# yjcaimeow/pointnerf

Hardware: AMD Instinct MI355X
Metric: Mray-samples/sec at 800x800, K=8, 2M neural points; PSNR delta vs ref (higher is better)
Workload: dtype fp32h2

## Files before the change

pointnerf_amd/csrc/aggregate_x3.hip:

```cpp
#include "agg_common.h"


namespace pnr {
namespace {

constexpr int kXT = 64;
constexpr int kXTS = kXT / kKN;
constexpr int kHidPlane = 32 * 64 * 16;
constexpr int kHidTile = 2 * kHidPlane;
constexpr int kXG = 34;
constexpr int kPG = 8;
constexpr int kPlaneX = kXG * kXT * 16;
constexpr int kPlaneP = kPG * kXT * 16;
constexpr int kP1Pitch = kHid + 4;

template <bool H>
struct XL {
  static constexpr int NPL = H ? 2 : 3;
  static constexpr int NPW = H ? 2 : 3;
  static constexpr unsigned kOne = H ? 0x3C00u : 0x3F80u;
  static constexpr int OffPE = NPL * kPlaneX;
  static constexpr int OffEx = OffPE + NPL * kPlaneP;
  static constexpr int NWB = H ? 3 : 2;
  static constexpr int OffWt = OffEx + 2 * 8 * kXT * 4;
  static constexpr int OffPr = OffWt + NWB * kXT * 4;
  static constexpr int OffSf = OffPr + 2 * kXT * 4;
  static constexpr int OffAp = OffSf + NWB * kXTS * 4;
  static constexpr int OffWa = OffAp + 4 * kXT * 4;
  static constexpr int OffH4 = OffWa + kHid * 4;
  static constexpr int OffTq = OffH4 + (H ? kXT * kP1Pitch * 4 : 0);
  static constexpr size_t Lds = (size_t)OffTq + 16;
  static_assert(OffSf % 16 == 0 && OffWa % 16 == 0 && OffH4 % 16 == 0, "16-B aligned LDS arrays");
  static_assert(kXT * kP1Pitch * 4 <= NPL * kPlaneX, "parked P1 fits the layer-input area");
  static_assert(Lds <= 160 * 1024, "LDS budget");
};

constexpr int kProducerPrio = 3;
constexpr int kStoreWindowPrio = 0;

typedef float f32x2n __attribute__((ext_vector_type(2)));
typedef float f32x4n __attribute__((ext_vector_type(4)));

struct X3Args {
  pnr_points pts;
  pnr_samples s;
  pnr_mlp w;
  SplitW wx;
  const float* p1;
  float* hid;
  int32_t* vmask;
  float* out_feat;
  float* out_weight;
  float* out_conf;
  int32_t* tile_ctr;
  pnr_agg_saved sv;
};

__device__ __forceinline__ bool xcd_mode(int64_t nt) { return nt >= 2 * (int64_t)gridDim.x + 16; }
__device__ __forceinline__ int64_t xcd_lo(int64_t nt, int x) { return nt * x / 8; }
__device__ __forceinline__ int64_t xcd_nb(int x) { return ((int)gridDim.x - x + 7) / 8; }

__device__ __forceinline__ int64_t first_tile(int64_t nt) {
  if (!xcd_mode(nt)) return blockIdx.x;
  return xcd_lo(nt, blockIdx.x & 7) + (blockIdx.x >> 3);
}

__device__ __forceinline__ int64_t take_tile(const X3Args& A, int64_t nt) {
  if (!xcd_mode(nt)) return (int64_t)gridDim.x + atomicAdd(A.tile_ctr, 1);
  const int x0 = blockIdx.x & 7;
  for (int i = 0; i < 8; ++i) {
    const int x = (x0 + i) & 7;
    const int64_t t = xcd_lo(nt, x) + xcd_nb(x) + atomicAdd(A.tile_ctr + x, 1);
    if (t < xcd_lo(nt, x + 1)) return t;
  }
  return nt;
}

__device__ __forceinline__ __amdgpu_buffer_rsrc_t rsrc(const void* base) {
  return __builtin_amdgcn_make_buffer_rsrc(const_cast<void*>(base), 0, 0x7fffffff, 0x00020000);
}

template <bool H, int NTK = 8>
__device__ __forceinline__ void load_w(uint4 (&a)[2][XL<H>::NPW], __amdgpu_buffer_rsrc_t rs, int voff, int t) {
  constexpr int NPW = XL<H>::NPW;
#pragma unroll
  for (int T = 0; T < 2; ++T)
#pragma unroll
    for (int pl = 0; pl < NPW; ++pl)
      a[T][pl] = __builtin_bit_cast(
          uint4, __builtin_amdgcn_raw_buffer_load_b128(
                     rs, voff + pl * 1024, (t * NTK + T) * NPW * 1024, 0));
}

template <bool H>
struct WRing {
  static constexpr int kWD = 3;
  uint4 a[kWD][2][XL<H>::NPW];
};

template <bool H, int NTK = 8>
__device__ __forceinline__ void prime(WRing<H>& w, __amdgpu_buffer_rsrc_t rs, int voff) {
#pragma unroll
  for (int d = 0; d < WRing<H>::kWD; ++d) load_w<H, NTK>(w.a[d], rs, voff, d);
}

template <bool H, int NTK = 8, bool ACC2 = false, bool ZACC = false>
__device__ __forceinline__ void layer(f32x16 (&acc)[4], f32x16 (&corr)[4], WRing<H>& w, __amdgpu_buffer_rsrc_t rs,
                                      int voff, const char* planes, int pstride, int nsteps, int lane) {
  static_assert(ACC2 || !ZACC, "zero-start accumulators: with two accumulator sets only");
  static_assert(H || !ACC2, "two accumulator sets: the f16 split only");
  constexpr int NPL = XL<H>::NPL, NPW = XL<H>::NPW, kWD = WRing<H>::kWD;
  const int c = lane & 31, h = lane >> 5;
  const char* base = planes + (h * kXT + c) * 16;
  auto ldb = [&](int t, int pt, uint4 (&bb)[NPL]) {
#pragma unroll
    for (int pl = 0; pl < NPL; ++pl)
      bb[pl] = *reinterpret_cast<const uint4*>(base + pl * pstride + (2 * t * kXT + 32 * pt) * 16);
  };
  constexpr int BD = H ? 2 : 1;
  uint4 b[BD][2][NPL];
#pragma unroll
  for (int sl = 0; sl < BD; ++sl) {
    const int t0 = sl < nsteps ? sl : nsteps - 1;
    ldb(t0, 0, b[sl][0]);
    ldb(t0, 1, b[sl][1]);
  }
  auto mm = [&](int pt, const uint4& av0, const uint4& av1, const uint4& bv, bool to_corr = false, bool zc = false) {
    if constexpr (ACC2) {
      f32x16 (&d)[4] = to_corr ? corr : acc;
      const f32x16 z = {0.f};
      d[2 * pt] = mfma_f16(av0, bv, zc ? z : d[2 * pt]);
      d[2 * pt + 1] = mfma_f16(av1, bv, zc ? z : d[2 * pt + 1]);
    } else if constexpr (H) {
      acc[2 * pt] = mfma_f16(av0, bv, acc[2 * pt]);
      acc[2 * pt + 1] = mfma_f16(av1, bv, acc[2 * pt + 1]);
    } else {
      acc[2 * pt] = mfma_bf16(av0, bv, acc[2 * pt]);
      acc[2 * pt + 1] = mfma_bf16(av1, bv, acc[2 * pt + 1]);
    }
  };
  auto wl = [&](uint4 (&a)[2][NPW], int pl, int tw) {
#pragma unroll
    for (int T = 0; T < 2; ++T)
      a[T][pl] = __builtin_bit_cast(
          uint4, __builtin_amdgcn_raw_buffer_load_b128(
                     rs, voff + pl * 1024, (tw * NTK + T) * NPW * 1024, 0));
  };
  auto bl = [&](int bs, int tn, int pt, int pl) {
    b[bs][pt][pl] = *reinterpret_cast<const uint4*>(base + pl * pstride + (2 * tn * kXT + 32 * pt) * 16);
  };
  uint4 scl[2];
  auto scale_next = [&](const uint4 (&an)[2][NPW], int T) {
    if constexpr (!ACC2) scl[T] = f16x8_scale2048(an[T][0]);
  };
  if constexpr (H) {
    scale_next(w.a[0], 0);
    scale_next(w.a[0], 1);
  }
  auto step_h = [&](uint4 (&a)[2][NPW], const uint4 (&an)[2][NPW], int t, int bs, bool first = false) {
    const int tn = t + BD < nsteps ? t + BD : nsteps - 1;
    const uint4 s0 = ACC2 ? a[0][0] : scl[0], s1 = ACC2 ? a[1][0] : scl[1];
#pragma unroll
    for (int pt = 0; pt < 2; ++pt) {
      mm(pt, s0, s1, b[bs][pt][0], false, first && ZACC);
      __builtin_amdgcn_sched_barrier(0);
      mm(pt, a[0][1], a[1][1], b[bs][pt][0], true, first);
      __builtin_amdgcn_sched_barrier(0);
      if (pt == 1) wl(a, 1, t + kWD);
      if (pt == 0) scale_next(an, 0);
      bl(bs, tn, pt, 0);
      __builtin_amdgcn_sched_barrier(0);
      mm(pt, a[0][0], a[1][0], b[bs][pt][1], true);
      __builtin_amdgcn_sched_barrier(0);
      bl(bs, tn, pt, 1);
      if (pt == 0) scale_next(an, 1);
      if (pt == 1) wl(a, 0, t + kWD);
      __builtin_amdgcn_sched_barrier(0);
    }
  };
  auto step = [&](uint4 (&a)[2][NPW], const uint4 (&an)[2][NPW], int t, int bs) {
    if constexpr (H) {
      step_h(a, an, t, bs);
    } else {
      const int tn = t + BD < nsteps ? t + BD : nsteps - 1;
#pragma unroll
      for (int pt = 0; pt < 2; ++pt) {
        mm(pt, a[0][2], a[1][2], b[bs][pt][0]);
        __builtin_amdgcn_sched_barrier(0);
        if (pt == 1) wl(a, 2, t + kWD);
        __builtin_amdgcn_sched_barrier(0);
        mm(pt, a[0][1], a[1][1], b[bs][pt][1]);
        mm(pt, a[0][0], a[1][0], b[bs][pt][2]);
        __builtin_amdgcn_sched_barrier(0);
        bl(bs, tn, pt, 2);
        __builtin_amdgcn_sched_barrier(0);
        mm(pt, a[0][1], a[1][1], b[bs][pt][0]);
        __builtin_amdgcn_sched_barrier(0);
        if (pt == 1) wl(a, 1, t + kWD);
        __builtin_amdgcn_sched_barrier(0);
        mm(pt, a[0][0], a[1][0], b[bs][pt][1]);
        __builtin_amdgcn_sched_barrier(0);
        bl(bs, tn, pt, 1);
        __builtin_amdgcn_sched_barrier(0);
        mm(pt, a[0][0], a[1][0], b[bs][pt][0]);
        __builtin_amdgcn_sched_barrier(0);
        bl(bs, tn, pt, 0);
        if (pt == 1) wl(a, 0, t + kWD);
        __builtin_amdgcn_sched_barrier(0);
      }
    }
  };
  constexpr int U = (BD == 2 && kWD % 2) ? 2 * kWD : kWD;
  constexpr int P = ACC2 ? 1 : 0;
  if constexpr (ACC2) step_h(w.a[0], w.a[1 % kWD], 0, 0, true);
  int t = P;
#pragma unroll 1
  for (; t + U <= nsteps; t += U) {
#pragma unroll
    for (int d = 0; d < U; ++d) step(w.a[(d + P) % kWD], w.a[(d + P + 1) % kWD], t + d, (d + P) % BD);
  }
#pragma unroll
  for (int d = 0; d < U - 1; ++d)
    if (t + d < nsteps) step(w.a[(d + P) % kWD], w.a[(d + P + 1) % kWD], t + d, (d + P) % BD);
}

template <bool H, int NTK = 8>
__device__ __forceinline__ void layer(f32x16 (&acc)[4], WRing<H>& w, __amdgpu_buffer_rsrc_t rs, int voff,
                                      const char* planes, int pstride, int nsteps, int lane) {
  layer<H, NTK, false>(acc, acc, w, rs, voff, planes, pstride, nsteps, lane);
}

__device__ __forceinline__ float fold2(float main, float corr) { return fmaf(main, 2048.f, corr); }

__device__ __forceinline__ void lrelu_splith(float x0, float x1, float k, float ks, unsigned& hi, unsigned& lo) {
  typedef float f2 __attribute__((ext_vector_type(2)));
  const f2 x = {x0, x1};
  const f2 Y = __builtin_elementwise_max(x * k, x * ks);
  asm volatile(
      "v_fma_mixlo_f16 %0, %2, %4, 0\n\t"
      "v_fma_mixhi_f16 %0, %3, %4, 0\n\t"
      "v_fma_mixlo_f16 %1, %0, %5, %2 op_sel_hi:[1,0,0]\n\t"
      "v_fma_mixhi_f16 %1, %0, %5, %3 op_sel:[1,0,0] op_sel_hi:[1,0,0]"
      : "=&v"(hi), "=&v"(lo)
      : "v"(Y.x), "v"(Y.y), "s"(0x1p-11f), "s"(-2048.f));
}

template <bool H, bool ACC2 = false>
__device__ __forceinline__ void store_act(const f32x16 (&acc)[4], const f32x16 (&corr)[4], char* planes, float s,
                                          float mul, int lane, int T0, int pstride = kPlaneX) {
  const int c = lane & 31, h = lane >> 5;
  if constexpr (H) {
    const float k = 2048.f * mul, ks = k * s;
#pragma unroll
    for (int pt = 0; pt < 2; ++pt)
#pragma unroll
      for (int T = 0; T < 2; ++T)
#pragma unroll
        for (int q = 0; q < 4; ++q) {
          float v[4];
#pragma unroll
          for (int i = 0; i < 4; ++i)
            v[i] = ACC2 ? fold2(acc[2 * pt + T][4 * q + i], corr[2 * pt + T][4 * q + i]) : acc[2 * pt + T][4 * q + i];
          unsigned a0, a1, b0, b1;
          lrelu_splith(v[0], v[1], k, ks, a0, a1);
          lrelu_splith(v[2], v[3], k, ks, b0, b1);
          char* d = planes + ((4 * (T0 + T) + q) * kXT + 32 * pt + c) * 16 + 8 * h;
          *reinterpret_cast<uint2*>(d) = make_uint2(a0, b0);
          *reinterpret_cast<uint2*>(d + pstride) = make_uint2(a1, b1);
        }
    return;
  }
#pragma unroll
  for (int pt = 0; pt < 2; ++pt)
#pragma unroll
    for (int T = 0; T < 2; ++T)
#pragma unroll
      for (int q = 0; q < 4; ++q) {
        const f32x16& v = acc[2 * pt + T];
        unsigned a0, a1, a2, b0, b1, b2;
        split2(fmaxf(v[4 * q], s * v[4 * q]), fmaxf(v[4 * q + 1], s * v[4 * q + 1]), a0, a1, a2);
        split2(fmaxf(v[4 * q + 2], s * v[4 * q + 2]), fmaxf(v[4 * q + 3], s * v[4 * q + 3]), b0, b1, b2);
        char* d = planes + ((4 * (T0 + T) + q) * kXT + 32 * pt + c) * 16 + 8 * h;
        *reinterpret_cast<uint2*>(d) = make_uint2(a0, b0);
        *reinterpret_cast<uint2*>(d + kPlaneX) = make_uint2(a1, b1);
        *reinterpret_cast<uint2*>(d + 2 * kPlaneX) = make_uint2(a2, b2);
      }
}

template <bool H>
__device__ __forceinline__ void store_act(const f32x16 (&acc)[4], char* planes, float s, float mul, int lane,
                                          int T0, int pstride = kPlaneX) {
  store_act<H, false>(acc, acc, planes, s, mul, lane, T0, pstride);
}

template <bool H>
__device__ __forceinline__ void acc_init(f32x16 (&acc)[4], const float* bias, float inv_scale, int lane, int T0) {
  if constexpr (H) {
    const int h = lane >> 5;
#pragma unroll
    for (int T = 0; T < 2; ++T)
#pragma unroll
      for (int q = 0; q < 4; ++q) {
        const float4 b = *reinterpret_cast<const float4*>(bias + 32 * (T0 + T) + 8 * q + 4 * h);
        const float v[4] = {b.x * inv_scale, b.y * inv_scale, b.z * inv_scale, b.w * inv_scale};
#pragma unroll
        for (int i = 0; i < 4; ++i) {
          acc[T][4 * q + i] = v[i];
          acc[2 + T][4 * q + i] = v[i];
        }
      }
  } else {
#pragma unroll
    for (int i = 0; i < 4; ++i) acc[i] = (f32x16){0.f};
  }
}
constexpr int kBiasSteps(bool H) { return H ? 16 : 17; }

template <bool H>
__device__ __forceinline__ void store_group(char* planes, int pstride, int g, int pair, const float (&v)[8]) {
  if constexpr (H) {
    uint4 p0, p1;
    splith(v[0], v[1], p0.x, p1.x);
    splith(v[2], v[3], p0.y, p1.y);
    splith(v[4], v[5], p0.z, p1.z);
    splith(v[6], v[7], p0.w, p1.w);
    char* d = planes + (g * kXT + pair) * 16;
    *reinterpret_cast<uint4*>(d) = p0;
    *reinterpret_cast<uint4*>(d + pstride) = p1;
    return;
  }
  uint4 p0, p1, p2;
  split2(v[0], v[1], p0.x, p1.x, p2.x);
  split2(v[2], v[3], p0.y, p1.y, p2.y);
  split2(v[4], v[5], p0.z, p1.z, p2.z);
  split2(v[6], v[7], p0.w, p1.w, p2.w);
  char* d = planes + (g * kXT + pair) * 16;
  *reinterpret_cast<uint4*>(d) = p0;
  *reinterpret_cast<uint4*>(d + pstride) = p1;
  *reinterpret_cast<uint4*>(d + 2 * pstride) = p2;
}

struct GatherState {
  int64_t tile;
  int64_t row;
  int pid;
  float sw[3], sp[3];
  int64_t dmap;
  bool active;
};

__device__ __forceinline__ void gather_row(const X3Args& A, int64_t tile, int lane, GatherState& g) {
  const int64_t v = tile * kXTS + (lane >> 3);
  g.tile = tile;
  g.active = v < eff_n(A.s);
  g.row = g.active ? sample_row(A.s, v) : 0;
}

__device__ __forceinline__ void gather_sample(const X3Args& A, int lane, GatherState& g) {
  const int k = lane & 7, K = A.s.K;
  g.pid = (g.active && k < K) ? A.s.pidx[g.row * K + k] : -1;
#pragma unroll
  for (int a = 0; a < 3; ++a) {
    g.sw[a] = g.active ? A.s.sample_w[g.row * 3 + a] : 0.f;
    g.sp[a] = g.active ? A.s.sample_p[g.row * 3 + a] : 0.f;
  }
  g.dmap = A.s.dir_map ? (int64_t)A.s.dir_map[g.row] : g.row;
}

template <bool H, bool TR = false>
__device__ __forceinline__ void gather(const X3Args& A, const GatherState& g, int nb, int nw, char* lds, int pw, int lane,
                                       float (&dr6)[6]) {
  using L = XL<H>;
  float Rw[9];
#pragma unroll
  for (int i = 0; i < 9; ++i) Rw[i] = A.w.rw2c ? A.w.rw2c[i] : (i % 4 == 0 ? 1.f : 0.f);
  float cam_c[3] = {0.f, 0.f, 0.f}, cam_R[9] = {1.f, 0.f, 0.f, 0.f, 1.f, 0.f, 0.f, 0.f, 1.f};
  if (!A.pts.pers) {
#pragma unroll
    for (int i = 0; i < 3; ++i) cam_c[i] = A.pts.campos[i];
#pragma unroll
    for (int i = 0; i < 9; ++i) cam_R[i] = A.pts.camrot[i];
  }
  const int j = lane >> 3, k = lane & 7;
  const int K = A.s.K;
  const bool active = g.active;
  const int64_t row = g.row;
  const bool valid = g.pid >= 0;
  const int64_t prow = valid ? g.pid : (active && k < K ? 0 : -1);
  float sw[3], sp[3], vd[3] = {0.f, 0.f, 0.f};
#pragma unroll
  for (int a = 0; a < 3; ++a) {
    sw[a] = g.sw[a];
    sp[a] = g.sp[a];
  }
  const int64_t drow = active ? g.dmap / A.s.dir_div : 0;
  if (active && pw == 0) {
#pragma unroll
    for (int a = 0; a < 3; ++a) vd[a] = A.s.dirs[drow * 3 + a];
  }
  float pw3[3] = {0.f, 0.f, 0.f}, pp[3] = {0.f, 0.f, 0.f}, col[3] = {0.f, 0.f, 0.f}, pdir[3] = {0.f, 0.f, 0.f};
  float cf = 1.f;
  if (valid) {
#pragma unroll
    for (int a = 0; a < 3; ++a) pw3[a] = A.pts.xyz[prow * 3 + a];
    if (pw == 0) {
#pragma unroll
      for (int a = 0; a < 3; ++a) {
        col[a] = A.pts.color ? A.pts.color[prow * 3 + a] : 0.f;
        pdir[a] = A.pts.dir ? A.pts.dir[prow * 3 + a] : 0.f;
      }
    }
    if (A.pts.pers) {
#pragma unroll
      for (int a = 0; a < 3; ++a) pp[a] = A.pts.pers[prow * 3 + a];
    } else {
      pair_pers(A.pts, A.s, drow, pw3, cam_c, cam_R, pp);
    }
  }
  if (pw == 0 && A.pts.conf && prow >= 0) cf = A.pts.conf[prow];
  float d6[6];
  d6[0] = pw3[0] - sw[0];
  d6[1] = pw3[1] - sw[1];
  d6[2] = pw3[2] - sw[2];
  d6[3] = pp[0] * pp[2] - sp[0] * sp[2];
  d6[4] = pp[1] * pp[2] - sp[1] * sp[2];
  d6[5] = pp[2] - sp[2];
  mat3(Rw, d6, dr6);
  dr6[3] = d6[3];
  dr6[4] = d6[4];
  dr6[5] = d6[5];
  if (A.pts.rw2c) rot_point(A.pts.rw2c, prow, d6, dr6);
  if (pw == 0) {
    const float nrm = sqrtf(d6[0] * d6[0] + d6[1] * d6[1] + d6[2] * d6[2]);
    const float wl = valid ? 1.f / fmaxf(nrm, 1e-6f) : 0.f;
    const float wsum = xor8_sum(wl);
    const float wn = wl / fmaxf(wsum, 1e-8f);
    const float confc = fminf(fmaxf(cf, 1e-4f), 1.f);
    const bool samp_valid = xor8_sum(valid ? 1.f : 0.f) > 0.f;
    float vrot[3], drot[3];
    mat3(Rw, vd, vrot);
    mat3(Rw, pdir, drot);
    if (A.pts.rw2c) {
      rot_point(A.pts.rw2c, prow, pdir, drot);
      rot_point(A.pts.rw2c, active ? slot0_point(A.s, row) : 0, vd, vrot);
    }
    const float dot = drot[0] * vrot[0] + drot[1] * vrot[1] + drot[2] * vrot[2];
    const float ex[8] = {col[0], col[1], col[2], drot[0] - vrot[0], drot[1] - vrot[1], drot[2] - vrot[2], dot, 1.f};
    float* exL = reinterpret_cast<float*>(lds + L::OffEx) + nb * 8 * kXT;
#pragma unroll
    for (int e = 0; e < 8; ++e) exL[e * kXT + lane] = ex[e];
    reinterpret_cast<float*>(lds + L::OffWt)[nw * kXT + lane] = wn * confc;
    reinterpret_cast<int*>(lds + L::OffPr)[nb * kXT + lane] = valid ? (int)prow : -1;
    if (k == 0) reinterpret_cast<int*>(lds + L::OffSf)[nw * kXTS + j] = active && samp_valid;
    if (active && k < K) {
      if (A.out_weight) A.out_weight[row * K + k] = wn;
      if (A.out_conf) A.out_conf[row * K + k] = confc;
    }
    if (TR && active) {
      const int64_t pr = g.tile * kXT + lane;
      float4* x = reinterpret_cast<float4*>(A.sv.x3e + pr * 32);
      x[0] = make_float4(ex[0], ex[1], ex[2], ex[3]);
      x[1] = make_float4(ex[4], ex[5], ex[6], ex[7]);
#pragma unroll
      for (int e = 2; e < 8; ++e) x[e] = make_float4(0.f, 0.f, 0.f, 0.f);
      A.sv.wt[pr] = wn * confc;
      A.sv.wn[pr] = wn;
      A.sv.prow[pr] = valid ? (int32_t)prow : -1;
    }
  }
}

template <bool H>
__device__ __forceinline__ void pe_store(char* lds, int lane, int e, float sn, float cs) {
  using L = XL<H>;
  const int r = 2 * e;
  char* d = lds + L::OffPE + ((r >> 3) * kXT + lane) * 16 + 2 * (r & 7);
  if constexpr (H) {
    unsigned x0, x1;
    splith(sn, cs, x0, x1);
    *reinterpret_cast<unsigned*>(d) = x0;
    *reinterpret_cast<unsigned*>(d + kPlaneP) = x1;
  } else {
    unsigned x0, x1, x2;
    split2(sn, cs, x0, x1, x2);
    *reinterpret_cast<unsigned*>(d) = x0;
    *reinterpret_cast<unsigned*>(d + kPlaneP) = x1;
    *reinterpret_cast<unsigned*>(d + 2 * kPlaneP) = x2;
  }
}

template <bool H, int PART, bool TR = false>
__device__ __forceinline__ void pe_planes(char* lds, int pw, int lane, const float (&dr6)[6],
                                          const X3Args* A = nullptr, const GatherState* g = nullptr) {
  using L = XL<H>;
  float* pe5 = TR && g->active ? A->sv.pe5 + (g->tile * kXT + lane) * 64 : nullptr;
  if (pw == 0 && PART == 0) {
    char* pz = lds + L::OffPE + (7 * kXT + lane) * 16 + 8;
#pragma unroll
    for (int pl = 0; pl < L::NPL; ++pl) *reinterpret_cast<uint2*>(pz + pl * kPlaneP) = make_uint2(0u, 0u);
    if (TR && pe5) *reinterpret_cast<float4*>(pe5 + 60) = make_float4(0.f, 0.f, 0.f, 0.f);
  }
  const int mine = __builtin_amdgcn_readfirstlane(PART == 0 ? pw : 4 + pw);
#pragma unroll
  for (int ch = 4 * PART; ch < (PART == 0 ? 4 : 6); ++ch) {
    if (ch != mine) continue;
    float s0, c0, s1, c1, s2, c2, s3, c3, s4, c4;
    sincosf(dr6[ch], &s0, &c0);
    sincosf(dr6[ch] * 2.f, &s1, &c1);
    sincosf(dr6[ch] * 4.f, &s2, &c2);
    sincosf(dr6[ch] * 8.f, &s3, &c3);
    sincosf(dr6[ch] * 16.f, &s4, &c4);
    pe_store<H>(lds, lane, 5 * ch + 0, s0, c0);
    pe_store<H>(lds, lane, 5 * ch + 1, s1, c1);
    pe_store<H>(lds, lane, 5 * ch + 2, s2, c2);
    pe_store<H>(lds, lane, 5 * ch + 3, s3, c3);
    pe_store<H>(lds, lane, 5 * ch + 4, s4, c4);
    if (TR && pe5) {
      const float sv[10] = {s0, c0, s1, c1, s2, c2, s3, c3, s4, c4};
#pragma unroll
      for (int i = 0; i < 10; i += 2) *reinterpret_cast<float2*>(pe5 + 10 * ch + i) = make_float2(sv[i], sv[i + 1]);
    }
  }
}

#define X3_SYNC() __syncthreads()

template <bool H, bool TR = false>
__device__ __forceinline__ void finalize_alpha(const X3Args& A, char* lds, int buf, int64_t tile, int lane) {
  using L = XL<H>;
  const int64_t n = eff_n(A.s);
  const int j = lane >> 3, k = lane & 7;
  const float* apart = reinterpret_cast<const float*>(lds + L::OffAp);
  const float* wtL = reinterpret_cast<const float*>(lds + L::OffWt) + buf * kXT;
  const int* sflag = reinterpret_cast<const int*>(lds + L::OffSf) + buf * kXTS;
  const float pa = apart[lane] + apart[kXT + lane] + apart[2 * kXT + lane] + apart[3 * kXT + lane] + A.w.ba[0];
  const float alpha_k = A.w.act_super ? softplus(pa - 1.f) : fmaxf(pa, 0.f);
  const float alpha_s = xor8_sum(wtL[lane] * alpha_k);
  const int64_t vo = tile * kXTS + j;
  if (TR && vo < n) A.sv.pa[tile * kXT + lane] = pa;
  if (k == 0 && vo < n) {
    A.vmask[vo] = sflag[j];
    if (sflag[j]) A.out_feat[vo * (kC + 1)] = alpha_s;
  }
}

template <bool H>
__device__ __forceinline__ void save_act_train(const X3Args& A, const f32x16 (&acc)[4], float* dst, int layer,
                                               int64_t tile, int64_t n, float neg, int lane, int T0, float sc) {
  const int c = lane & 31, h = lane >> 5;
#pragma unroll
  for (int pt = 0; pt < 2; ++pt) {
    const int col = 32 * pt + c;
    if (tile * kXTS + (col >> 3) >= n) continue;
    const int64_t pr = tile * kXT + col;
#pragma unroll
    for (int T = 0; T < 2; ++T) {
      f32x16 v = acc[2 * pt + T];
      if constexpr (H) v = v * sc;
      unsigned bits = 0;
#pragma unroll
      for (int q = 0; q < 4; ++q)
        *reinterpret_cast<float4*>(dst + pr * kHid + 32 * (T0 + T) + 8 * q + 4 * h) =
            make_float4(lrelu(v[4 * q], neg), lrelu(v[4 * q + 1], neg), lrelu(v[4 * q + 2], neg),
                        lrelu(v[4 * q + 3], neg));
#pragma unroll
      for (int r = 0; r < 16; ++r) bits |= (v[r] > 0.f ? 1u : 0u) << r;
      A.sv.mask[pr * 64 + 16 * layer + 2 * (T0 + T) + h] = (uint16_t)bits;
    }
  }
}

template <bool H, bool TR = false>
__device__ __forceinline__ void consumer_loop(const X3Args& A, char* lds, int wid, int lane) {
  using L = XL<H>;
  const int c = lane & 31, h = lane >> 5;
  const int64_t n = eff_n(A.s);
  const int64_t ntiles = cdiv(n, kXTS);
  const float neg = A.w.neg_slope;
  char* XP = lds;
  const char* PE = lds + L::OffPE;
  const float* P1L = reinterpret_cast<const float*>(lds);
  float* apart = reinterpret_cast<float*>(lds + L::OffAp);
  const float* waL = reinterpret_cast<const float*>(lds + L::OffWa);
  const int T0 = 2 * wid;
  const int voff = (T0 * L::NPW * 64 + lane) * 16;
  const __amdgpu_buffer_rsrc_t r1 = rsrc(A.wx.pack[0]), r2 = rsrc(A.wx.pack[1]), r3 = rsrc(A.wx.pack[2]),
                               r4 = rsrc(A.wx.pack[3]);
  const float sc1 = A.wx.scale[0], sc2 = A.wx.scale[1], sc3 = A.wx.scale[2], sc4 = A.wx.scale[3];
  constexpr bool A2 = H && !TR;
  const float in2 = A2 ? 0x1p-11f : 1.f;
  WRing<H> wr;
  f32x16 acc[4];
  f32x16 corr[4];
  auto zero_acc = [&]() {
    if constexpr (!A2) {
#pragma unroll
      for (int i = 0; i < 4; ++i) acc[i] = (f32x16){0.f};
    }
  };
  prime<H>(wr, r1, voff);
  X3_SYNC();
  const int* TQ = reinterpret_cast<const int*>(lds + L::OffTq);
  int it = 0;
  for (int64_t tile = first_tile(ntiles); tile < ntiles; tile = TQ[(it + 1) & 3], ++it) {
    const int buf = it & 1;
    zero_acc();
    layer<H, 8, A2, A2>(acc, corr, wr, r1, voff, PE, kPlaneP, 4, lane);
    prime<H>(wr, r2, voff);
    X3_SYNC();
#pragma unroll
    for (int pt = 0; pt < 2; ++pt)
#pragma unroll
      for (int T = 0; T < 2; ++T)
#pragma unroll
        for (int q = 0; q < 4; ++q) {
          const float4 v4 = *reinterpret_cast<const float4*>(P1L + (32 * pt + c) * kP1Pitch + 32 * (T0 + T) + 8 * q +
                                                             4 * h);
          if constexpr (A2) {
            const float v[4] = {v4.x, v4.y, v4.z, v4.w};
#pragma unroll
            for (int i = 0; i < 4; ++i)
              acc[2 * pt + T][4 * q + i] =
                  fmaf(acc[2 * pt + T][4 * q + i], 2048.f * sc1, fmaf(corr[2 * pt + T][4 * q + i], sc1, v[i]));
          } else if constexpr (H) {
            acc[2 * pt + T][4 * q] = fmaf(acc[2 * pt + T][4 * q], sc1, v4.x);
            acc[2 * pt + T][4 * q + 1] = fmaf(acc[2 * pt + T][4 * q + 1], sc1, v4.y);
            acc[2 * pt + T][4 * q + 2] = fmaf(acc[2 * pt + T][4 * q + 2], sc1, v4.z);
            acc[2 * pt + T][4 * q + 3] = fmaf(acc[2 * pt + T][4 * q + 3], sc1, v4.w);
          } else {
            acc[2 * pt + T][4 * q] += v4.x;
            acc[2 * pt + T][4 * q + 1] += v4.y;
            acc[2 * pt + T][4 * q + 2] += v4.z;
            acc[2 * pt + T][4 * q + 3] += v4.w;
          }
        }
    X3_SYNC();
    store_act<H>(acc, XP, neg, 1.f, lane, T0);
    if constexpr (TR) save_act_train<H>(A, acc, A.sv.h1, 0, tile, n, neg, lane, T0, 1.f);
    if (wid == 0) {
#pragma unroll
      for (int pl = 0; pl < L::NPL; ++pl) {
        *reinterpret_cast<uint4*>(XP + pl * kPlaneX + (32 * kXT + lane) * 16) =
            make_uint4(pl == 0 ? L::kOne : 0u, 0u, 0u, 0u);
        *reinterpret_cast<uint4*>(XP + pl * kPlaneX + (33 * kXT + lane) * 16) = make_uint4(0u, 0u, 0u, 0u);
      }
    }
    acc_init<H>(acc, A.w.b2, in2 / sc2, lane, T0);
    X3_SYNC();
    layer<H, 8, A2>(acc, corr, wr, r2, voff, XP, kPlaneX, kBiasSteps(H), lane);
    prime<H>(wr, r3, voff);
    X3_SYNC();
    store_act<H, A2>(acc, corr, XP, neg, sc2, lane, T0);
    if constexpr (TR) save_act_train<H>(A, acc, A.sv.h2, 1, tile, n, neg, lane, T0, sc2);
    if (wid == 0) {
      const float* exL = reinterpret_cast<const float*>(lds + L::OffEx) + buf * 8 * kXT;
      float ex[8];
#pragma unroll
      for (int e = 0; e < 8; ++e) ex[e] = exL[e * kXT + lane];
      store_group<H>(XP, kPlaneX, 32, lane, ex);
    }
    zero_acc();
    X3_SYNC();
    layer<H, 8, A2, A2>(acc, corr, wr, r3, voff, XP, kPlaneX, 17, lane);
    prime<H>(wr, r4, voff);
    X3_SYNC();
    store_act<H, A2>(acc, corr, XP, neg, sc3, lane, T0);
    if constexpr (TR) save_act_train<H>(A, acc, A.sv.h3, 2, tile, n, neg, lane, T0, sc3);
    if (wid == 0 && !H) {
#pragma unroll
      for (int pl = 0; pl < L::NPL; ++pl)
        *reinterpret_cast<uint4*>(XP + pl * kPlaneX + (32 * kXT + lane) * 16) =
            make_uint4(pl == 0 ? L::kOne : 0u, 0u, 0u, 0u);
    }
    acc_init<H>(acc, A.w.b4, in2 / sc4, lane, T0);
    X3_SYNC();
    layer<H, 8, A2>(acc, corr, wr, r4, voff, XP, kPlaneX, kBiasSteps(H), lane);
    prime<H>(wr, r1, voff);
    if constexpr (H) {
      if constexpr (TR) save_act_train<H>(A, acc, A.sv.h4, 3, tile, n, neg, lane, T0, sc4);
      float* H4 = reinterpret_cast<float*>(lds + L::OffH4);
#pragma unroll
      for (int pt = 0; pt < 2; ++pt)
#pragma unroll
        for (int T = 0; T < 2; ++T)
#pragma unroll
          for (int q = 0; q < 4; ++q) {
            float v[4];
#pragma unroll
            for (int i = 0; i < 4; ++i)
              v[i] = A2 ? fold2(acc[2 * pt + T][4 * q + i], corr[2 * pt + T][4 * q + i]) : acc[2 * pt + T][4 * q + i];
            *reinterpret_cast<float4*>(H4 + (32 * pt + c) * kP1Pitch + 32 * (T0 + T) + 8 * q + 4 * h) =
                make_float4(v[0], v[1], v[2], v[3]);
          }
    } else {
      if constexpr (TR) save_act_train<H>(A, acc, A.sv.h4, 3, tile, n, neg, lane, T0, 1.f);
      const float* wtL = reinterpret_cast<const float*>(lds + L::OffWt) + buf * kXT;
      const int* sflag = reinterpret_cast<const int*>(lds + L::OffSf) + buf * kXTS;
      float pa_part[2] = {0.f, 0.f};
      const int i8 = c & 7;
      const bool b2 = (i8 & 4) != 0, b1 = (i8 & 2) != 0, b0 = (i8 & 1) != 0;
#pragma unroll
      for (int pt = 0; pt < 2; ++pt) {
        const float wtp = wtL[32 * pt + c];
        const int sj = (32 * pt + c) >> 3;
        const int64_t vo = tile * kXTS + sj;
        const bool wrt = vo < n && sflag[sj];
#pragma unroll
        for (int T = 0; T < 2; ++T) {
          float v[16];
#pragma unroll
          for (int r = 0; r < 16; ++r) {
            const float hv = lrelu(H ? acc[2 * pt + T][r] * sc4 : acc[2 * pt + T][r], neg);
            pa_part[pt] += waL[32 * (T0 + T) + acc_row(r, h)] * hv;
            v[r] = wtp * hv;
          }
          float w8[8], w4[4], w2[2];
#pragma unroll
          for (int q = 0; q < 8; ++q) {
            const float send = b2 ? v[q] : v[q + 8];
            const float recv = __builtin_bit_cast(
                float, __builtin_amdgcn_mov_dpp(__builtin_bit_cast(int, send), 0x141, 0xf, 0xf, false));
            w8[q] = (b2 ? v[q + 8] : v[q]) + recv;
          }
#pragma unroll
          for (int q = 0; q < 4; ++q) {
            const float send = b1 ? w8[q] : w8[q + 4];
            const float recv = __builtin_bit_cast(
                float, __builtin_amdgcn_mov_dpp(__builtin_bit_cast(int, send), 0x4E, 0xf, 0xf, false));
            w4[q] = (b1 ? w8[q + 4] : w8[q]) + recv;
          }
#pragma unroll
          for (int q = 0; q < 2; ++q) {
            const float send = b0 ? w4[q] : w4[q + 2];
            const float recv = __builtin_bit_cast(
                float, __builtin_amdgcn_mov_dpp(__builtin_bit_cast(int, send), 0xB1, 0xf, 0xf, false));
            w2[q] = (b0 ? w4[q + 2] : w4[q]) + recv;
          }
          if (wrt)
            __builtin_nontemporal_store(
                (f32x2n){w2[0], w2[1]},
                reinterpret_cast<f32x2n*>(A.hid + vo * kHid + 32 * (T0 + T) + ((2 * i8) & 3) + 8 * (i8 >> 1) + 4 * h));
        }
        pa_part[pt] += __shfl_xor(pa_part[pt], 32);
      }
      if (h == 0) {
        apart[wid * kXT + c] = pa_part[0];
        apart[wid * kXT + 32 + c] = pa_part[1];
      }
    }
    X3_SYNC();
  }
}

__device__ __forceinline__ unsigned fetch_p1(f32x4n (&r)[16], const X3Args& A, const int* prow, int pw, int lane) {
  int64_t rows[16];
#pragma unroll
  for (int i = 0; i < 16; ++i) {
    const int pr = prow[16 * pw + i];
    rows[i] = pr < 0 ? -1 : (A.pts.used_map ? (int64_t)A.pts.used_map[pr] : (int64_t)pr);
  }
  unsigned empty = 0;
#pragma unroll
  for (int i = 0; i < 16; ++i) {
    r[i] = __builtin_nontemporal_load(reinterpret_cast<const f32x4n*>(A.p1 + (rows[i] < 0 ? 0 : rows[i]) * kHid) +
                                      lane);
    if (rows[i] < 0) empty |= 1u << i;
  }
  return empty;
}

__device__ __forceinline__ void park_p1(const f32x4n (&r)[16], unsigned empty, char* lds, int pw, int lane) {
  float* P1L = reinterpret_cast<float*>(lds);
#pragma unroll
  for (int i = 0; i < 16; ++i) {
    const f32x4n z = {0.f, 0.f, 0.f, 0.f};
    *reinterpret_cast<f32x4n*>(P1L + (16 * pw + i) * kP1Pitch + 4 * lane) = ((empty >> i) & 1) ? z : r[i];
  }
}

struct TailState {
  float hs[8], pa[8];
};

template <int PART, bool TR = false>
__device__ __forceinline__ void producer_tail(const X3Args& A, char* lds, int slot, int64_t tile, int pw, int lane,
                                              TailState& ts, float& chk) {
  using L = XL<true>;
  const int64_t n = eff_n(A.s);
  const int j = 2 * pw + (lane >> 5), ng = lane & 31;
  const float* H4 = reinterpret_cast<const float*>(lds + L::OffH4);
  const float* wtL = reinterpret_cast<const float*>(lds + L::OffWt) + slot * kXT + 8 * j;
  const int sf = reinterpret_cast<const int*>(lds + L::OffSf)[slot * kXTS + j];
  const float* waL = reinterpret_cast<const float*>(lds + L::OffWa) + 8 * ng;
  const float sc = A.wx.scale[3], neg = A.w.neg_slope;
  const float4 wa0 = *reinterpret_cast<const float4*>(waL), wa1 = *reinterpret_cast<const float4*>(waL + 4);
  const float wa[8] = {wa0.x, wa0.y, wa0.z, wa0.w, wa1.x, wa1.y, wa1.z, wa1.w};
  const float4 wt0 = *reinterpret_cast<const float4*>(wtL), wt1 = *reinterpret_cast<const float4*>(wtL + 4);
  const float wt[8] = {wt0.x, wt0.y, wt0.z, wt0.w, wt1.x, wt1.y, wt1.z, wt1.w};
  float (&hs)[8] = ts.hs;
  float (&pa)[8] = ts.pa;
#pragma unroll
  for (int k = 4 * PART; k < 4 * PART + 4; ++k) {
    const float* row = H4 + (8 * j + k) * kP1Pitch + 8 * ng;
    const float4 a = *reinterpret_cast<const float4*>(row), b = *reinterpret_cast<const float4*>(row + 4);
    const float x[8] = {a.x, a.y, a.z, a.w, b.x, b.y, b.z, b.w};
    float p = 0.f;
#pragma unroll
    for (int i = 0; i < 8; ++i) {
      const float hv = lrelu(x[i] * sc, neg);
      p = fmaf(wa[i], hv, p);
      hs[i] = k == 0 ? wt[0] * hv : fmaf(wt[k], hv, hs[i]);
    }
    pa[k] = p;
  }
  if (PART == 0) return;
  const bool b4 = (ng & 16) != 0, b3 = (ng & 8) != 0, b2 = (ng & 4) != 0;
  float r4[4], r2[2];
#pragma unroll
  for (int q = 0; q < 4; ++q) r4[q] = (b4 ? pa[q + 4] : pa[q]) + __shfl_xor(b4 ? pa[q] : pa[q + 4], 16);
#pragma unroll
  for (int q = 0; q < 2; ++q) r2[q] = (b3 ? r4[q + 2] : r4[q]) + __shfl_xor(b3 ? r4[q] : r4[q + 2], 8);
  float r1 = (b2 ? r2[1] : r2[0]) + __shfl_xor(b2 ? r2[0] : r2[1], 4);
  r1 += __shfl_xor(r1, 2);
  r1 += __shfl_xor(r1, 1);
  const float pk = r1 + A.w.ba[0];
  if (TR && (ng & 3) == 0 && tile * kXTS + j < n) A.sv.pa[tile * kXT + 8 * j + (ng >> 2)] = pk;
  const float alpha_k = A.w.act_super ? softplus(pk - 1.f) : fmaxf(pk, 0.f);
  float as = wtL[ng >> 2] * alpha_k;
  as += __shfl_xor(as, 4);
  as += __shfl_xor(as, 8);
  as += __shfl_xor(as, 16);
  chk = fmaf(0.f, (hs[0] + hs[1]) + (hs[2] + hs[3]) + (hs[4] + hs[5]) + (hs[6] + hs[7]) + as, chk);
  const int64_t vo = tile * kXTS + j;
  if (vo < n) {
    if (ng == 0) {
      A.vmask[vo] = sf;
      if (sf) A.out_feat[vo * (kC + 1)] = as;
    }
    if (TR) {
      if (sf) {
        float4* dst = reinterpret_cast<float4*>(A.hid + vo * kHid + 8 * ng);
        dst[0] = make_float4(hs[0], hs[1], hs[2], hs[3]);
        dst[1] = make_float4(hs[4], hs[5], hs[6], hs[7]);
      }
    } else if (sf) {
      typedef unsigned u32x4n __attribute__((ext_vector_type(4)));
      unsigned a[4], b[4];
#pragma unroll
      for (int i = 0; i < 4; ++i) splith(hs[2 * i], hs[2 * i + 1], a[i], b[i]);
      const u32x4n p0 = {a[0], a[1], a[2], a[3]}, p1 = {b[0], b[1], b[2], b[3]};
      u32x4n* dst = reinterpret_cast<u32x4n*>(reinterpret_cast<char*>(A.hid) + (vo / kXT) * kHidTile +
                                              (ng * kXT + vo % kXT) * 16);
      dst[0] = p0;
      dst[kHidPlane / 16] = p1;
    }
  }
}

template <bool H, bool TR = false>
__device__ __forceinline__ void producer_loop(const X3Args& A, char* lds, int pw, int lane) {
  using L = XL<H>;
  constexpr bool SW = H && !TR;
  const int64_t n = eff_n(A.s);
  const int64_t ntiles = cdiv(n, kXTS);
  __builtin_amdgcn_s_setprio(kProducerPrio);
  f32x4n p1r[16];
  unsigned p1e = 0;
  float dr6[6];
  GatherState g;
  gather_row(A, first_tile(ntiles), lane, g);
  gather_sample(A, lane, g);
  gather<H, TR>(A, g, 0, 0, lds, pw, lane, dr6);
  pe_planes<H, 0, TR>(lds, pw, lane, dr6, &A, &g);
  pe_planes<H, 1, TR>(lds, pw, lane, dr6, &A, &g);
  int* TQ = reinterpret_cast<int*>(lds + L::OffTq);
  if (pw == 0 && lane == 0) TQ[1] = (int)take_tile(A, ntiles);
  X3_SYNC();
  p1e = fetch_p1(p1r, A, reinterpret_cast<const int*>(lds + L::OffPr), pw, lane);
  X3_SYNC();
  float chk = 0.f;
  TailState ts;
  int it = 0;
  int64_t prev = -1;
  for (int64_t tile = first_tile(ntiles); tile < ntiles; prev = tile, tile = TQ[(it + 1) & 3], ++it) {
    const int nbuf = (it & 1) ^ 1;
    const int nw = H ? (it + 1) % 3 : nbuf;
    const int64_t next = TQ[(it + 1) & 3];
    if (pw == 0 && lane == 0) TQ[(it + 2) & 3] = next < ntiles ? (int)take_tile(A, ntiles) : (int)ntiles;
    park_p1(p1r, p1e, lds, pw, lane);
    gather_row(A, next, lane, g);
    X3_SYNC();
    if (!H && pw == 0 && it > 0) finalize_alpha<H, TR>(A, lds, nbuf, prev, lane);
    X3_SYNC();
    gather_sample(A, lane, g);
    X3_SYNC();
    gather<H, TR>(A, g, nbuf, nw, lds, pw, lane, dr6);
    if constexpr (H)
      if (it > 0) producer_tail<0, TR>(A, lds, (it + 2) % 3, prev, pw, lane, ts, chk);
    X3_SYNC();
    p1e = fetch_p1(p1r, A, reinterpret_cast<const int*>(lds + L::OffPr) + nbuf * kXT, pw, lane);
    X3_SYNC();
    if constexpr (!SW) pe_planes<H, 0, TR>(lds, pw, lane, dr6, &A, &g);
    if constexpr (H)
      if (it > 0) producer_tail<1, TR>(A, lds, (it + 2) % 3, prev, pw, lane, ts, chk);
    X3_SYNC();
    if constexpr (SW) {
      __builtin_amdgcn_s_setprio(kStoreWindowPrio);
      pe_planes<H, 0, TR>(lds, pw, lane, dr6, &A, &g);
      __builtin_amdgcn_s_setprio(kProducerPrio);
    }
    X3_SYNC();
    pe_planes<H, 1, TR>(lds, pw, lane, dr6, &A, &g);
    X3_SYNC();
  }
  if constexpr (H) {
    if (it > 0) {
      producer_tail<0, TR>(A, lds, (it - 1) % 3, prev, pw, lane, ts, chk);
      producer_tail<1, TR>(A, lds, (it - 1) % 3, prev, pw, lane, ts, chk);
    }
    if (A.wx.range_flag && chk != 0.f) atomicOr(A.wx.range_flag, 1);
  } else {
    if (pw == 0 && it > 0) finalize_alpha<H, TR>(A, lds, (it - 1) & 1, prev, lane);
  }
}

template <bool H, bool TR = false>
__device__ __forceinline__ void pairs_body(const X3Args& A) {
  extern __shared__ __attribute__((aligned(16))) char lds[];
  const int lane = threadIdx.x & 63, wid = threadIdx.x >> 6;
  if (threadIdx.x < kHid) reinterpret_cast<float*>(lds + XL<H>::OffWa)[threadIdx.x] = A.w.wa[threadIdx.x];
  if (wid < 4) {
    X3_SYNC();
    consumer_loop<H, TR>(A, lds, wid, lane);
  } else {
    producer_loop<H, TR>(A, lds, wid - 4, lane);
  }
}

__global__ void __launch_bounds__(512, 1) k_pairs_x3(X3Args A) { pairs_body<false>(A); }
__global__ void __launch_bounds__(512, 1) k_pairs_h2(X3Args A) { pairs_body<true>(A); }
__global__ void __launch_bounds__(512, 1) k_pairs_x3_train(X3Args A) { pairs_body<false, true>(A); }
__global__ void __launch_bounds__(512, 1) k_pairs_h2_train(X3Args A) { pairs_body<true, true>(A); }

constexpr int kCG = 18;
constexpr int kCPlane = kCG * kXT * 16;
constexpr size_t kColH2Lds = 2 * (size_t)kCPlane;
constexpr int kOPitch = kC + 4;
static_assert((size_t)kXT * kOPitch * 4 <= kColH2Lds, "output staging must fit the planes");

struct ColH2Args {
  pnr_samples s;
  pnr_mlp w;
  const void* pack[4];
  float scale[3];
  int32_t* range_flag;
  const float* hid;
  const int32_t* vmask;
  float* out_feat;
  const float* rw2c_pp;
  const float* hid_rows;
  float* vpe;
  float* hc[3];
};

template <int G0, int NG>
__device__ __forceinline__ void color_load_hid(const ColH2Args& A, char* lds, int64_t tile) {
  const int lane = threadIdx.x & 63, pl = threadIdx.x >> 6;
  const char* src = reinterpret_cast<const char*>(A.hid) + tile * kHidTile + lane * 16;
#pragma unroll
  for (int g = 0; g < NG; ++g) {
    __builtin_amdgcn_global_load_lds(
        (const __attribute__((address_space(1))) void*)(src + pl * kHidPlane + (G0 + g) * kXT * 16),
        (__attribute__((address_space(3))) void*)(lds + pl * kCPlane + g * kXT * 16), 16, 0, 0);
  }
}

template <int G0, int NG>
__device__ __forceinline__ void color_split_hid(const ColH2Args& A, char* lds, int64_t tile, int64_t n) {
  const int lane = threadIdx.x & 63, wid = threadIdx.x >> 6;
  const int64_t v = tile * kXT + lane;
  const bool ok = v < n;
  const float4* src = reinterpret_cast<const float4*>(A.hid_rows + (ok ? v : 0) * kHid);
#pragma unroll
  for (int gg = 0; gg < (NG + 1) / 2; ++gg) {
    const int g = 2 * gg + wid;
    if (g >= NG) break;
    const float4 a = ok ? src[2 * (G0 + g)] : make_float4(0.f, 0.f, 0.f, 0.f);
    const float4 b = ok ? src[2 * (G0 + g) + 1] : make_float4(0.f, 0.f, 0.f, 0.f);
    const float g8[8] = {a.x, a.y, a.z, a.w, b.x, b.y, b.z, b.w};
    store_group<true>(lds, kCPlane, g, lane, g8);
  }
}

__device__ __forceinline__ void save_act_rows(const f32x16 (&acc)[4], float* dst, int64_t v0, int64_t n, float neg,
                                              float scale, int lane, int T0) {
  const int c = lane & 31, h = lane >> 5;
#pragma unroll
  for (int pt = 0; pt < 2; ++pt) {
    const int64_t v = v0 + 32 * pt + c;
    if (v >= n) continue;
#pragma unroll
    for (int T = 0; T < 2; ++T)
#pragma unroll
      for (int q = 0; q < 4; ++q) {
        const f32x16& a = acc[2 * pt + T];
        *reinterpret_cast<float4*>(dst + v * kC + 32 * (T0 + T) + 8 * q + 4 * h) =
            make_float4(lrelu(a[4 * q] * scale, neg), lrelu(a[4 * q + 1] * scale, neg),
                        lrelu(a[4 * q + 2] * scale, neg), lrelu(a[4 * q + 3] * scale, neg));
      }
  }
}

template <bool TR>
__global__ void __launch_bounds__(128) __attribute__((amdgpu_waves_per_eu(2, 2))) k_color_h2(ColH2Args A) {
  extern __shared__ __attribute__((aligned(16))) char lds[];
  const int lane = threadIdx.x & 63, wid = threadIdx.x >> 6;
  const int c = lane & 31, h = lane >> 5;
  const int64_t n = eff_n(A.s);
  const int64_t ntiles = cdiv(n, kXT);
  const float neg = A.w.neg_slope;
  float Rw[9];
#pragma unroll
  for (int i = 0; i < 9; ++i) Rw[i] = A.w.rw2c ? A.w.rw2c[i] : (i % 4 == 0 ? 1.f : 0.f);
  const int T0 = 2 * wid;
  const int voff = (T0 * XL<true>::NPW * 64 + lane) * 16;
  const __amdgpu_buffer_rsrc_t r1a = rsrc(A.pack[0]), r1b = rsrc(A.pack[1]), r2 = rsrc(A.pack[2]),
                               r3 = rsrc(A.pack[3]);
  float chk = 0.f;
  WRing<true> wr;
  f32x16 acc[4];
  prime<true, 4>(wr, r1a, voff);
  for (int64_t tile = blockIdx.x; tile < ntiles; tile += gridDim.x) {
    const int64_t v0 = tile * kXT;
    const uint64_t vm = __ballot(v0 + lane < n && A.vmask[v0 + lane] != 0);
    if constexpr (TR) color_split_hid<0, kCG>(A, lds, tile, n);
    else color_load_hid<0, kCG>(A, lds, tile);
    __syncthreads();
#pragma unroll
    for (int i = 0; i < 4; ++i) acc[i] = (f32x16){0.f};
    layer<true, 4>(acc, wr, r1a, voff, lds, kCPlane, 9, lane);
    prime<true, 4>(wr, r1b, voff);
    __syncthreads();
    if constexpr (TR) color_split_hid<kCG, 14>(A, lds, tile, n);
    else color_load_hid<kCG, 14>(A, lds, tile);
    if (wid == 0) {
      const int64_t v = v0 + lane;
      float vrot[3] = {0.f, 0.f, 0.f};
      if (v < n) {
        const int64_t row = sample_row(A.s, v);
        const int64_t drow = dir_row(A.s, row);
        const float vd[3] = {A.s.dirs[drow * 3], A.s.dirs[drow * 3 + 1], A.s.dirs[drow * 3 + 2]};
        mat3(Rw, vd, vrot);
        if (A.rw2c_pp) rot_point(A.rw2c_pp, slot0_point(A.s, row), vd, vrot);
      }
      float pe[32];
#pragma unroll
      for (int ch = 0; ch < 3; ++ch)
#pragma unroll
        for (int f = 0; f < 4; ++f) {
          float sn, cs;
          sincosf(vrot[ch] * (float)(1 << f), &sn, &cs);
          pe[4 * ch + f] = sn;
          pe[12 + 4 * ch + f] = cs;
        }
      if (TR && v < n) {
#pragma unroll
        for (int i = 0; i < 24; ++i) A.vpe[v * 24 + i] = pe[i];
      }
      pe[24] = 1.f;
#pragma unroll
      for (int i = 25; i < 32; ++i) pe[i] = 0.f;
#pragma unroll
      for (int q = 0; q < 4; ++q) {
        const float g8[8] = {pe[8 * q], pe[8 * q + 1], pe[8 * q + 2], pe[8 * q + 3],
                             pe[8 * q + 4], pe[8 * q + 5], pe[8 * q + 6], pe[8 * q + 7]};
        store_group<true>(lds, kCPlane, 14 + q, lane, g8);
      }
    }
    __syncthreads();
    layer<true, 4>(acc, wr, r1b, voff, lds, kCPlane, 9, lane);
    prime<true, 4>(wr, r2, voff);
    __syncthreads();
    if (TR) save_act_rows(acc, A.hc[0], v0, n, neg, A.scale[0], lane, T0);
// ... 244 lines not shown
```

Before: 841.9.

## Gather once per tile in wave 0 and share rotated offsets through LDS

In the fp16 inference path, only producer wave 0 now runs the neighbour gather and rotation. It writes the six rotated offset channels to LDS, and the other producer waves read them to compute their positional-encoding sincos planes. Previously every producer wave repeated the gather. The change also precomputes the scaled layer-2 and layer-4 biases into LDS once per block, and folds the output scale into the alpha and weight coefficients in the tail. The cost is more LDS use, and a load imbalance because wave 0 now carries all the gather latency.

```diff
diff --git a/pointnerf_amd/csrc/aggregate_x3.hip b/pointnerf_amd/csrc/aggregate_x3.hip
--- a/pointnerf_amd/csrc/aggregate_x3.hip
+++ b/pointnerf_amd/csrc/aggregate_x3.hip
@@ -29,8 +29,10 @@
   static constexpr int OffWa = OffAp + 4 * kXT * 4;
   static constexpr int OffH4 = OffWa + kHid * 4;
   static constexpr int OffTq = OffH4 + (H ? kXT * kP1Pitch * 4 : 0);
-  static constexpr size_t Lds = (size_t)OffTq + 16;
-  static_assert(OffSf % 16 == 0 && OffWa % 16 == 0 && OffH4 % 16 == 0, "16-B aligned LDS arrays");
+  static constexpr int OffBi = OffTq + 16;
+  static constexpr int OffD6 = OffBi + (H ? 2 * kHid * 4 : 0);
+  static constexpr size_t Lds = (size_t)OffD6 + (H ? 6 * kXT * 4 : 0);
+  static_assert(OffSf % 16 == 0 && OffWa % 16 == 0 && OffH4 % 16 == 0 && OffBi % 16 == 0, "16-B aligned LDS arrays");
   static_assert(kXT * kP1Pitch * 4 <= NPL * kPlaneX, "parked P1 fits the layer-input area");
   static_assert(Lds <= 160 * 1024, "LDS budget");
 };
@@ -314,6 +316,21 @@
     for (int i = 0; i < 4; ++i) acc[i] = (f32x16){0.f};
   }
 }
+__device__ __forceinline__ void acc_init_lds(f32x16 (&acc)[4], const float* bi, int lane, int T0) {
+  const int h = lane >> 5;
+#pragma unroll
+  for (int T = 0; T < 2; ++T)
+#pragma unroll
+    for (int q = 0; q < 4; ++q) {
+      const float4 b = *reinterpret_cast<const float4*>(bi + 32 * (T0 + T) + 8 * q + 4 * h);
+      const float v[4] = {b.x, b.y, b.z, b.w};
+#pragma unroll
+      for (int i = 0; i < 4; ++i) {
+        acc[T][4 * q + i] = v[i];
+        acc[2 + T][4 * q + i] = v[i];
+      }
+    }
+}
 constexpr int kBiasSteps(bool H) { return H ? 16 : 17; }
 
 template <bool H>
@@ -367,7 +384,7 @@
   g.dmap = A.s.dir_map ? (int64_t)A.s.dir_map[g.row] : g.row;
 }
 
-template <bool H, bool TR = false>
+template <bool H, bool TR = false, bool D6L = false>
 __device__ __forceinline__ void gather(const X3Args& A, const GatherState& g, int nb, int nw, char* lds, int pw, int lane,
                                        float (&dr6)[6]) {
   using L = XL<H>;
@@ -430,6 +447,11 @@
   dr6[4] = d6[4];
   dr6[5] = d6[5];
   if (A.pts.rw2c) rot_point(A.pts.rw2c, prow, d6, dr6);
+  if constexpr (D6L) {
+    float* d6L = reinterpret_cast<float*>(lds + L::OffD6);
+#pragma unroll
+    for (int i = 0; i < 6; ++i) d6L[i * kXT + lane] = dr6[i];
+  }
   if (pw == 0) {
     const float nrm = sqrtf(d6[0] * d6[0] + d6[1] * d6[1] + d6[2] * d6[2]);
     const float wl = valid ? 1.f / fmaxf(nrm, 1e-6f) : 0.f;
@@ -523,6 +545,30 @@
   }
 }
 
+template <int PART>
+__device__ __forceinline__ void pe_planes_lds(char* lds, int pw, int lane) {
+  using L = XL<true>;
+  if (pw == 0 && PART == 0) {
+    char* pz = lds + L::OffPE + (7 * kXT + lane) * 16 + 8;
+#pragma unroll
+    for (int pl = 0; pl < L::NPL; ++pl) *reinterpret_cast<uint2*>(pz + pl * kPlaneP) = make_uint2(0u, 0u);
+  }
+  if (PART == 1 && pw >= 2) return;
+  const int ch = __builtin_amdgcn_readfirstlane(PART == 0 ? pw : 4 + pw);
+  const float x = reinterpret_cast<const float*>(lds + L::OffD6)[ch * kXT + lane];
+  float s0, c0, s1, c1, s2, c2, s3, c3, s4, c4;
+  sincosf(x, &s0, &c0);
+  sincosf(x * 2.f, &s1, &c1);
+  sincosf(x * 4.f, &s2, &c2);
+  sincosf(x * 8.f, &s3, &c3);
+  sincosf(x * 16.f, &s4, &c4);
+  pe_store<true>(lds, lane, 5 * ch + 0, s0, c0);
+  pe_store<true>(lds, lane, 5 * ch + 1, s1, c1);
+  pe_store<true>(lds, lane, 5 * ch + 2, s2, c2);
+  pe_store<true>(lds, lane, 5 * ch + 3, s3, c3);
+  pe_store<true>(lds, lane, 5 * ch + 4, s4, c4);
+}
+
 #define X3_SYNC() __syncthreads()
 
 template <bool H, bool TR = false>
@@ -582,6 +628,7 @@
   const float* P1L = reinterpret_cast<const float*>(lds);
   float* apart = reinterpret_cast<float*>(lds + L::OffAp);
   const float* waL = reinterpret_cast<const float*>(lds + L::OffWa);
+  const float* biL = reinterpret_cast<const float*>(lds + L::OffBi);
   const int T0 = 2 * wid;
   const int voff = (T0 * L::NPW * 64 + lane) * 16;
   const __amdgpu_buffer_rsrc_t r1 = rsrc(A.wx.pack[0]), r2 = rsrc(A.wx.pack[1]), r3 = rsrc(A.wx.pack[2]),
@@ -645,7 +692,8 @@
         *reinterpret_cast<uint4*>(XP + pl * kPlaneX + (33 * kXT + lane) * 16) = make_uint4(0u, 0u, 0u, 0u);
       }
     }
-    acc_init<H>(acc, A.w.b2, in2 / sc2, lane, T0);
+    if constexpr (A2) acc_init_lds(acc, biL, lane, T0);
+    else acc_init<H>(acc, A.w.b2, in2 / sc2, lane, T0);
     X3_SYNC();
     layer<H, 8, A2>(acc, corr, wr, r2, voff, XP, kPlaneX, kBiasSteps(H), lane);
     prime<H>(wr, r3, voff);
@@ -672,7 +720,8 @@
         *reinterpret_cast<uint4*>(XP + pl * kPlaneX + (32 * kXT + lane) * 16) =
             make_uint4(pl == 0 ? L::kOne : 0u, 0u, 0u, 0u);
     }
-    acc_init<H>(acc, A.w.b4, in2 / sc4, lane, T0);
+    if constexpr (A2) acc_init_lds(acc, biL + kHid, lane, T0);
+    else acc_init<H>(acc, A.w.b4, in2 / sc4, lane, T0);
     X3_SYNC();
     layer<H, 8, A2>(acc, corr, wr, r4, voff, XP, kPlaneX, kBiasSteps(H), lane);
     prime<H>(wr, r1, voff);
@@ -794,9 +843,16 @@
   const float* waL = reinterpret_cast<const float*>(lds + L::OffWa) + 8 * ng;
   const float sc = A.wx.scale[3], neg = A.w.neg_slope;
   const float4 wa0 = *reinterpret_cast<const float4*>(waL), wa1 = *reinterpret_cast<const float4*>(waL + 4);
-  const float wa[8] = {wa0.x, wa0.y, wa0.z, wa0.w, wa1.x, wa1.y, wa1.z, wa1.w};
+  float wa[8] = {wa0.x, wa0.y, wa0.z, wa0.w, wa1.x, wa1.y, wa1.z, wa1.w};
   const float4 wt0 = *reinterpret_cast<const float4*>(wtL), wt1 = *reinterpret_cast<const float4*>(wtL + 4);
-  const float wt[8] = {wt0.x, wt0.y, wt0.z, wt0.w, wt1.x, wt1.y, wt1.z, wt1.w};
+  float wt[8] = {wt0.x, wt0.y, wt0.z, wt0.w, wt1.x, wt1.y, wt1.z, wt1.w};
+  constexpr bool FS = !TR;
+  if constexpr (FS) {
+#pragma unroll
+    for (int i = 0; i < 8; ++i) wa[i] *= sc;
+#pragma unroll
+    for (int k = 4 * PART; k < 4 * PART + 4; ++k) wt[k] *= sc;
+  }
   float (&hs)[8] = ts.hs;
   float (&pa)[8] = ts.pa;
 #pragma unroll
@@ -807,7 +863,7 @@
     float p = 0.f;
 #pragma unroll
     for (int i = 0; i < 8; ++i) {
-      const float hv = lrelu(x[i] * sc, neg);
+      const float hv = lrelu(FS ? x[i] : x[i] * sc, neg);
       p = fmaf(wa[i], hv, p);
       hs[i] = k == 0 ? wt[0] * hv : fmaf(wt[k], hv, hs[i]);
     }
@@ -868,15 +924,30 @@
   unsigned p1e = 0;
   float dr6[6];
   GatherState g;
-  gather_row(A, first_tile(ntiles), lane, g);
-  gather_sample(A, lane, g);
-  gather<H, TR>(A, g, 0, 0, lds, pw, lane, dr6);
-  pe_planes<H, 0, TR>(lds, pw, lane, dr6, &A, &g);
-  pe_planes<H, 1, TR>(lds, pw, lane, dr6, &A, &g);
+  constexpr bool G1 = SW;
+  const bool gw = !G1 || __builtin_amdgcn_readfirstlane(pw) == 0;
   int* TQ = reinterpret_cast<int*>(lds + L::OffTq);
-  if (pw == 0 && lane == 0) TQ[1] = (int)take_tile(A, ntiles);
-  X3_SYNC();
-  p1e = fetch_p1(p1r, A, reinterpret_cast<const int*>(lds + L::OffPr), pw, lane);
+  if constexpr (G1) {
+    if (gw) {
+      gather_row(A, first_tile(ntiles), lane, g);
+      gather_sample(A, lane, g);
+      gather<H, TR, true>(A, g, 0, 0, lds, 0, lane, dr6);
+    }
+    if (pw == 0 && lane == 0) TQ[1] = (int)take_tile(A, ntiles);
+    X3_SYNC();
+    p1e = fetch_p1(p1r, A, reinterpret_cast<const int*>(lds + L::OffPr), pw, lane);
+    pe_planes_lds<0>(lds, pw, lane);
+    pe_planes_lds<1>(lds, pw, lane);
+  } else {
+    gather_row(A, first_tile(ntiles), lane, g);
+    gather_sample(A, lane, g);
+    gather<H, TR>(A, g, 0, 0, lds, pw, lane, dr6);
+    pe_planes<H, 0, TR>(lds, pw, lane, dr6, &A, &g);
+    pe_planes<H, 1, TR>(lds, pw, lane, dr6, &A, &g);
+    if (pw == 0 && lane == 0) TQ[1] = (int)take_tile(A, ntiles);
+    X3_SYNC();
+    p1e = fetch_p1(p1r, A, reinterpret_cast<const int*>(lds + L::OffPr), pw, lane);
+  }
   X3_SYNC();
   float chk = 0.f;
   TailState ts;
@@ -888,13 +959,17 @@
     const int64_t next = TQ[(it + 1) & 3];
     if (pw == 0 && lane == 0) TQ[(it + 2) & 3] = next < ntiles ? (int)take_tile(A, ntiles) : (int)ntiles;
     park_p1(p1r, p1e, lds, pw, lane);
-    gather_row(A, next, lane, g);
+    if (gw) gather_row(A, next, lane, g);
     X3_SYNC();
     if (!H && pw == 0 && it > 0) finalize_alpha<H, TR>(A, lds, nbuf, prev, lane);
     X3_SYNC();
-    gather_sample(A, lane, g);
-    X3_SYNC();
-    gather<H, TR>(A, g, nbuf, nw, lds, pw, lane, dr6);
+    if (gw) gather_sample(A, lane, g);
+    X3_SYNC();
+    if constexpr (G1) {
+      if (gw) gather<H, TR, true>(A, g, nbuf, nw, lds, 0, lane, dr6);
+    } else {
+      gather<H, TR>(A, g, nbuf, nw, lds, pw, lane, dr6);
+    }
     if constexpr (H)
       if (it > 0) producer_tail<0, TR>(A, lds, (it + 2) % 3, prev, pw, lane, ts, chk);
     X3_SYNC();
@@ -906,11 +981,13 @@
     X3_SYNC();
     if constexpr (SW) {
       __builtin_amdgcn_s_setprio(kStoreWindowPrio);
-      pe_planes<H, 0, TR>(lds, pw, lane, dr6, &A, &g);
+      if constexpr (G1) pe_planes_lds<0>(lds, pw, lane);
+      else pe_planes<H, 0, TR>(lds, pw, lane, dr6, &A, &g);
       __builtin_amdgcn_s_setprio(kProducerPrio);
     }
     X3_SYNC();
-    pe_planes<H, 1, TR>(lds, pw, lane, dr6, &A, &g);
+    if constexpr (G1) pe_planes_lds<1>(lds, pw, lane);
+    else pe_planes<H, 1, TR>(lds, pw, lane, dr6, &A, &g);
     X3_SYNC();
   }
   if constexpr (H) {
@@ -929,6 +1006,13 @@
   extern __shared__ __attribute__((aligned(16))) char lds[];
   const int lane = threadIdx.x & 63, wid = threadIdx.x >> 6;
   if (threadIdx.x < kHid) reinterpret_cast<float*>(lds + XL<H>::OffWa)[threadIdx.x] = A.w.wa[threadIdx.x];
+  if constexpr (H && !TR) {
+    if (threadIdx.x < kHid) {
+      float* bi = reinterpret_cast<float*>(lds + XL<H>::OffBi);
+      bi[threadIdx.x] = A.w.b2[threadIdx.x] * (0x1p-11f / A.wx.scale[1]);
+      bi[kHid + threadIdx.x] = A.w.b4[threadIdx.x] * (0x1p-11f / A.wx.scale[3]);
+    }
+  }
   if (wid < 4) {
     X3_SYNC();
     consumer_loop<H, TR>(A, lds, wid, lane);
```

Measured after the change: 847.9, median of 6. Within noise of the previous version (+0.7%).
